# zxhuang1698/ZeroShape

Hardware: AMD Instinct MI355X
Metric: sdf_query_points_per_sec_vox128 (higher is better)
Workload: dtype f16x3

## Files before the change

### zeroshape_amd/csrc/sdf_prologue.hip

```cpp
#include "zs_common.h"
#include "sdf_layout.h"
#include "../../include/zeroshape_hip.h"

#include <math.h>

namespace {

using namespace zs::lay;

constexpr int ROWS = 4;
constexpr int LIN_THREADS = 256;
constexpr int KMAX = 1024;

__device__ __forceinline__ float wave_sum(float v) {
#pragma unroll
    for (int o = 32; o > 0; o >>= 1) v += __shfl_xor(v, o, 64);
    return v;
}

__device__ __forceinline__ float erf_ref(float x) { return erff(x); }

template <bool LN_IN, bool GELU, bool RESID, bool POS>
__global__ __launch_bounds__(LIN_THREADS) void lat_linear_kernel(
    const float *__restrict__ X, int ldx, size_t x_stride, int K, const float *__restrict__ Wt,
    const float *__restrict__ bias, int N, const float *__restrict__ ln_g,
    const float *__restrict__ ln_b, const float *__restrict__ resid, int ldr, size_t r_stride,
    const float *__restrict__ pos, float *__restrict__ Y, int ldy, size_t y_stride, int rows) {
    __shared__ float xs[ROWS][KMAX];
    const int img = blockIdx.z;
    const int r0 = blockIdx.x * ROWS;
    const int n = blockIdx.y * LIN_THREADS + threadIdx.x;
    X += (size_t)img * x_stride;
    Y += (size_t)img * y_stride;

    for (int i = threadIdx.x; i < ROWS * K; i += LIN_THREADS) {
        const int r = i / K, k = i - r * K;
        const int rr = min(r0 + r, rows - 1);
        xs[r][k] = X[(size_t)rr * ldx + k];
    }
    __syncthreads();
    if (LN_IN) {
        const int w = threadIdx.x >> 6, lane = threadIdx.x & 63;
        float v[4], s = 0.f;
#pragma unroll
        for (int j = 0; j < 4; j++) {
            v[j] = xs[w][lane + 64 * j];
            s += v[j];
        }
        const float mean = wave_sum(s) * (1.0f / 256.0f);
        float q = 0.f;
#pragma unroll
        for (int j = 0; j < 4; j++) {
            const float d = v[j] - mean;
            q = fmaf(d, d, q);
        }
        const float rstd = 1.0f / sqrtf(wave_sum(q) * (1.0f / 256.0f) + 1e-6f);
#pragma unroll
        for (int j = 0; j < 4; j++) {
            const int k = lane + 64 * j;
            xs[w][k] = fmaf((v[j] - mean) * rstd, ln_g[k], ln_b[k]);
        }
        __syncthreads();
    }
    float acc[ROWS];
#pragma unroll
    for (int r = 0; r < ROWS; r++) acc[r] = 0.f;
    for (int k0 = 0; k0 < K; k0 += 16) {
        float w[16];
#pragma unroll
        for (int j = 0; j < 16; j++) w[j] = Wt[(size_t)(k0 + j) * N + n];
#pragma unroll
        for (int j = 0; j < 16; j++)
#pragma unroll
            for (int r = 0; r < ROWS; r++) acc[r] = fmaf(xs[r][k0 + j], w[j], acc[r]);
    }
    const float b = bias[n];
#pragma unroll
    for (int r = 0; r < ROWS; r++) {
        const int row = r0 + r;
        if (row >= rows) break;
        float v = acc[r] + b;
        if (POS) v += pos[(size_t)row * N + n];
        if (GELU) v = 0.5f * v * (1.0f + erf_ref(v * 0.70710678118654752440f));
        if (RESID) v += resid[(size_t)img * r_stride + (size_t)row * ldr + n];
        Y[(size_t)row * ldy + n] = v;
    }
}

__global__ __launch_bounds__(256) void lat_self_attn_kernel(const float *__restrict__ qkv,
                                                            size_t stride, float *__restrict__ out,
                                                            size_t out_stride) {
    __shared__ float ks[L][HD];
    __shared__ float vs[L][HD];
    const int hd = blockIdx.x, img = blockIdx.y;
    qkv += (size_t)img * stride;
    out += (size_t)img * out_stride;
    for (int i = threadIdx.x; i < L * HD; i += 256) {
        const int r = i / HD, d = i - r * HD;
        ks[r][d] = qkv[(size_t)r * (3 * C) + C + hd * HD + d];
        vs[r][d] = qkv[(size_t)r * (3 * C) + 2 * C + hd * HD + d];
    }
    __syncthreads();
    const int i = threadIdx.x;
    if (i >= L) return;
    float q[HD], o[HD];
#pragma unroll
    for (int d = 0; d < HD; d++) {
        q[d] = qkv[(size_t)i * (3 * C) + hd * HD + d];
        o[d] = 0.f;
    }
    const float scale = 0.17677669529663688110f;
    float m = -INFINITY, z = 0.f;
    for (int j = 0; j < L; j++) {
        float s = 0.f;
#pragma unroll
        for (int d = 0; d < HD; d++) s = fmaf(q[d], ks[j][d], s);
        s *= scale;
        const float mn = fmaxf(m, s);
        const float a = expf(m - mn), p = expf(s - mn);
        z = fmaf(z, a, p);
#pragma unroll
        for (int d = 0; d < HD; d++) o[d] = fmaf(p, vs[j][d], o[d] * a);
        m = mn;
    }
    const float inv = 1.0f / z;
#pragma unroll
    for (int d = 0; d < HD; d++) out[(size_t)i * C + hd * HD + d] = o[d] * inv;
}

__global__ __launch_bounds__(256) void pack_kv_kernel(const float *__restrict__ scratch,
                                                      size_t scratch_stride,
                                                      float *__restrict__ programs,
                                                      size_t program_stride) {
    const int img = blockIdx.y;
    const int e = blockIdx.x * 256 + threadIdx.x;
    const int lane = e & 63;
    const int r = (e >> 6) & 15;
    const int which = (e >> 10) & 1;
    int t = e >> 11;
    const int lt = t % LT;
    t /= LT;
    const int hd = t & 7;
    const int blk = t >> 3;
    if (blk >= BLOCKS) return;
    const float *sc = scratch + (size_t)img * scratch_stride;
    const int rw = (r & 3) + 8 * (r >> 2) + 4 * (lane >> 5);
    const int lrow = 32 * lt + (which == 0 ? (lane & 31) : rw);
    const int dim = which == 0 ? rw : (lane & 31);
    float val = 0.f;
    if (lrow < L) {
        if (blk == 0)
            val = sc[S_QKV0 + (size_t)lrow * (3 * C) + (1 + which) * C + hd * HD + dim];
        else
            val = sc[S_KV1 + (size_t)lrow * (2 * C) + which * C + hd * HD + dim];
    }
    const int group = blk * G_BLOCK + hd * G_HEAD + G_QKV_HEAD + lt * 8 + which * 4 + (r >> 2);
    programs[(size_t)img * program_stride + (size_t)group * GROUP_FLOATS + lane * 4 + (r & 3)] = val;
}

template <bool LN_IN, bool GELU, bool RESID, bool POS>
void launch_linear(hipStream_t s, int batch, const float *X, int ldx, size_t x_stride, int K,
                   const float *Wt, const float *bias, int N, const float *g, const float *b,
                   const float *resid, int ldr, size_t r_stride, const float *pos, float *Y, int ldy,
                   size_t y_stride) {
    dim3 grid((L + ROWS - 1) / ROWS, N / LIN_THREADS, batch);
    hipLaunchKernelGGL((lat_linear_kernel<LN_IN, GELU, RESID, POS>), grid, dim3(LIN_THREADS), 0, s, X,
                       ldx, x_stride, K, Wt, bias, N, g, b, resid, ldr, r_stride, pos, Y, ldy,
                       y_stride, L);
}

}

__global__ __launch_bounds__(256) void verdict_stats_kernel(const float *__restrict__ got, const float *__restrict__ want, int m,
                                                            float band, float tol, float tol_occ, float *__restrict__ stats,
                                                            int *__restrict__ flags) {
    __shared__ float red[4][256];
    __shared__ int redi[2][256];
    const int b = blockIdx.x, t = threadIdx.x;
    const float *g = got + (size_t)b * m, *w = want + (size_t)b * m;
    float mx = 0.f, sum = 0.f, mw = 0.f, mo = 0.f;
    int flips = 0, bad = 0;
    for (int i = t; i < m; i += 256) {
        const float x = g[i], y = w[i];
        if (!isfinite(x) || !isfinite(y)) bad = 1;
        const float d = fabsf(x - y);
        mx = fmaxf(mx, d);
        sum += d;
        mw = fmaxf(mw, fabsf(y));
        mo = fmaxf(mo, fabsf(1.0f / (1.0f + expf(-x)) - 1.0f / (1.0f + expf(-y))));
        flips += ((x > 0.f) != (y > 0.f)) && fabsf(y) >= band;
    }
    red[0][t] = mx; red[1][t] = sum; red[2][t] = mw; red[3][t] = mo;
    redi[0][t] = flips; redi[1][t] = bad;
    __syncthreads();
    for (int o = 128; o > 0; o >>= 1) {
        if (t < o) {
            red[0][t] = fmaxf(red[0][t], red[0][t + o]);
            red[1][t] += red[1][t + o];
            red[2][t] = fmaxf(red[2][t], red[2][t + o]);
            red[3][t] = fmaxf(red[3][t], red[3][t + o]);
            redi[0][t] += redi[0][t + o];
            redi[1][t] |= redi[1][t + o];
        }
        __syncthreads();
    }
    if (t == 0) {
        const bool finite = redi[1][0] == 0;
        const float nan = __builtin_bit_cast(float, 0x7fc00000u);
        float *o = stats + (size_t)b * 5;
        o[0] = finite ? red[0][0] : nan;
        o[1] = finite ? red[1][0] / (float)m : nan;
        o[2] = finite ? red[2][0] : nan;
        o[3] = finite ? red[3][0] : nan;
        o[4] = (float)redi[0][0];
        if (flags) {
            flags[2 * b] = (finite && red[0][0] <= tol) ? 0 : 1;
            flags[2 * b + 1] = (finite && red[3][0] <= tol_occ && redi[0][0] == 0) ? 0 : 1;
        }
    }
}

extern "C" int zs_sdf_verdict_stats(const float *got, const float *want, int batch, int m, float flip_band, float tol,
                                    float tol_occ, float *stats, int *flags, void *stream) {
    if (batch < 0 || batch > 65535 || m <= 0) {
        zs::set_err("zs_sdf_verdict_stats: bad size (batch=%d m=%d)", batch, m);
        return 0;
    }
    if (batch == 0) return 1;
    if (!got || !want || !stats) {
        zs::set_err("zs_sdf_verdict_stats: null pointer");
        return 0;
    }
    hipLaunchKernelGGL(verdict_stats_kernel, dim3(batch), dim3(256), 0, static_cast<hipStream_t>(stream), got, want, m, flip_band,
                       tol, tol_occ, stats, flags);
    return zs::check_launch("zs_sdf_verdict_stats") ? 1 : 0;
}

extern "C" size_t zs_sdf_prologue_scratch_bytes(void) { return (size_t)SCRATCH_FLOATS * sizeof(float); }

extern "C" int zs_sdf_prologue(void *programs, size_t program_stride_bytes, const float *lat_params,
                               const float *latent_depth, int batch, void *scratch, void *stream) {
    return zs_sdf_prologue_ex(programs, program_stride_bytes, lat_params, latent_depth, batch, scratch, 0, stream);
}

extern "C" int zs_sdf_prologue_ex(void *programs, size_t program_stride_bytes, const float *lat_params,
                                  const float *latent_depth, int batch, void *scratch, int flags, void *stream) {
    if (flags & ~ZS_SDF_POS_PERLAYER) {
        zs::set_err("zs_sdf_prologue_ex: unknown flags 0x%x", flags);
        return 0;
    }
    if (batch < 0) {
        zs::set_err("zs_sdf_prologue: negative batch %d", batch);
        return 0;
    }
    if (batch == 0) return 1;
    if (!programs || !lat_params || !latent_depth || !scratch) {
        zs::set_err("zs_sdf_prologue: null pointer");
        return 0;
    }
    if (program_stride_bytes % 16 != 0 || program_stride_bytes < zs_sdf_program_bytes()) {
        zs::set_err("zs_sdf_prologue: bad program stride %zu", program_stride_bytes);
        return 0;
    }
    if (batch > 65535) {
        zs::set_err("zs_sdf_prologue: batch %d > 65535", batch);
        return 0;
    }
    hipStream_t s = static_cast<hipStream_t>(stream);
    const float *P = lat_params;
    float *sc = static_cast<float *>(scratch);
    const size_t ss = SCRATCH_FLOATS;
    launch_linear<false, false, false, true>(s, batch, latent_depth, C, (size_t)L * C, C, P + LQ_WLP,
                                             P + LQ_BLP, C, nullptr, nullptr, nullptr, 0, 0,
                                             P + LQ_POS, sc + S_LAT, C, ss);
    launch_linear<true, false, false, false>(s, batch, sc + S_LAT, C, ss, C, P + LQ_WQKV0,
                                             P + LQ_BQKV0, 3 * C, P + LQ_LN1G0, P + LQ_LN1B0, nullptr,
                                             0, 0, nullptr, sc + S_QKV0, 3 * C, ss);
    hipLaunchKernelGGL(lat_self_attn_kernel, dim3(HEADS, batch), dim3(256), 0, s, sc + S_QKV0, ss,
                       sc + S_ATT, ss);
    launch_linear<false, false, true, false>(s, batch, sc + S_ATT, C, ss, C, P + LQ_WPROJ0,
                                             P + LQ_BPROJ0, C, nullptr, nullptr, sc + S_LAT, C, ss,
                                             nullptr, sc + S_X1, C, ss);
    launch_linear<true, true, false, false>(s, batch, sc + S_X1, C, ss, C, P + LQ_W1, P + LQ_B1, HID,
                                            P + LQ_LN2G0, P + LQ_LN2B0, nullptr, 0, 0, nullptr,
                                            sc + S_HID, HID, ss);
    if (flags & ZS_SDF_POS_PERLAYER)
        launch_linear<false, false, true, true>(s, batch, sc + S_HID, HID, ss, HID, P + LQ_W2, P + LQ_B2,
                                                C, nullptr, nullptr, sc + S_X1, C, ss, P + LQ_POS,
                                                sc + S_X2, C, ss);
    else
        launch_linear<false, false, true, false>(s, batch, sc + S_HID, HID, ss, HID, P + LQ_W2, P + LQ_B2,
                                                 C, nullptr, nullptr, sc + S_X1, C, ss, nullptr,
                                                 sc + S_X2, C, ss);
    launch_linear<true, false, false, false>(s, batch, sc + S_X2, C, ss, C, P + LQ_WKV1, P + LQ_BKV1,
                                             2 * C, P + LQ_LN1G1, P + LQ_LN1B1, nullptr, 0, 0, nullptr,
                                             sc + S_KV1, 2 * C, ss);
    const int elems = BLOCKS * HEADS * LT * 2 * 16 * 64;
    hipLaunchKernelGGL(pack_kv_kernel, dim3((elems + 255) / 256, batch), dim3(256), 0, s, sc, ss,
                       static_cast<float *>(programs), program_stride_bytes / sizeof(float));
    return zs::check_launch("zs_sdf_prologue") ? 1 : 0;
}
```

Baseline: 84.92 million.

## Fuse latent prologue linears into three kernels with direct KV packing

Replaces the chain of separate linear launches plus a pack kernel with three kernels: a fused projection+LN+QKV kernel, a row-tiled self-attention kernel that precomputes scores and softmax factors in LDS, and a fused proj+MLP+LN+KV kernel that writes packed KV directly into the program buffer. Weight loads are double-buffered in registers. The aim is to cut launch count, intermediate scratch round-trips and the serial per-thread attention loop. The cost is heavier per-block register use, and the prologue runs once per batch, so its share of the query throughput metric may be small.

```diff
diff --git a/zeroshape_amd/csrc/sdf_prologue.hip b/zeroshape_amd/csrc/sdf_prologue.hip
--- a/zeroshape_amd/csrc/sdf_prologue.hip
+++ b/zeroshape_amd/csrc/sdf_prologue.hip
@@ -8,9 +8,23 @@
 
 using namespace zs::lay;
 
-constexpr int ROWS = 4;
+#ifndef ZS_PROLOGUE_ROWS
+#define ZS_PROLOGUE_ROWS 4
+#endif
+constexpr int ROWS = ZS_PROLOGUE_ROWS;
 constexpr int LIN_THREADS = 256;
-constexpr int KMAX = 1024;
+constexpr int ROW_BLOCKS = (L + ROWS - 1) / ROWS;
+constexpr int LROWS_REC = LT * 32;
+
+#ifndef ZS_PROLOGUE_LOADS
+#define ZS_PROLOGUE_LOADS 32
+#endif
+
+constexpr int chunk_rows(int nc) {
+    int d = 1;
+    while (2 * d * nc <= ZS_PROLOGUE_LOADS) d *= 2;
+    return d;
+}
 
 __device__ __forceinline__ float wave_sum(float v) {
 #pragma unroll
@@ -20,27 +34,10 @@
 
 __device__ __forceinline__ float erf_ref(float x) { return erff(x); }
 
-template <bool LN_IN, bool GELU, bool RESID, bool POS>
-__global__ __launch_bounds__(LIN_THREADS) void lat_linear_kernel(
-    const float *__restrict__ X, int ldx, size_t x_stride, int K, const float *__restrict__ Wt,
-    const float *__restrict__ bias, int N, const float *__restrict__ ln_g,
-    const float *__restrict__ ln_b, const float *__restrict__ resid, int ldr, size_t r_stride,
-    const float *__restrict__ pos, float *__restrict__ Y, int ldy, size_t y_stride, int rows) {
-    __shared__ float xs[ROWS][KMAX];
-    const int img = blockIdx.z;
-    const int r0 = blockIdx.x * ROWS;
-    const int n = blockIdx.y * LIN_THREADS + threadIdx.x;
-    X += (size_t)img * x_stride;
-    Y += (size_t)img * y_stride;
-
-    for (int i = threadIdx.x; i < ROWS * K; i += LIN_THREADS) {
-        const int r = i / K, k = i - r * K;
-        const int rr = min(r0 + r, rows - 1);
-        xs[r][k] = X[(size_t)rr * ldx + k];
-    }
-    __syncthreads();
-    if (LN_IN) {
-        const int w = threadIdx.x >> 6, lane = threadIdx.x & 63;
+__device__ __forceinline__ void layer_norm_rows(float (*xs)[C], const float *__restrict__ ln_g,
+                                                const float *__restrict__ ln_b) {
+    const int lane = threadIdx.x & 63;
+    for (int w = threadIdx.x >> 6; w < ROWS; w += LIN_THREADS / 64) {
         float v[4], s = 0.f;
 #pragma unroll
         for (int j = 0; j < 4; j++) {
@@ -60,113 +57,247 @@
             const int k = lane + 64 * j;
             xs[w][k] = fmaf((v[j] - mean) * rstd, ln_g[k], ln_b[k]);
         }
-        __syncthreads();
-    }
-    float acc[ROWS];
-#pragma unroll
-    for (int r = 0; r < ROWS; r++) acc[r] = 0.f;
-    for (int k0 = 0; k0 < K; k0 += 16) {
-        float w[16];
-#pragma unroll
-        for (int j = 0; j < 16; j++) w[j] = Wt[(size_t)(k0 + j) * N + n];
-#pragma unroll
-        for (int j = 0; j < 16; j++)
-#pragma unroll
-            for (int r = 0; r < ROWS; r++) acc[r] = fmaf(xs[r][k0 + j], w[j], acc[r]);
-    }
-    const float b = bias[n];
-#pragma unroll
-    for (int r = 0; r < ROWS; r++) {
-        const int row = r0 + r;
-        if (row >= rows) break;
-        float v = acc[r] + b;
-        if (POS) v += pos[(size_t)row * N + n];
-        if (GELU) v = 0.5f * v * (1.0f + erf_ref(v * 0.70710678118654752440f));
-        if (RESID) v += resid[(size_t)img * r_stride + (size_t)row * ldr + n];
-        Y[(size_t)row * ldy + n] = v;
-    }
-}
-
-__global__ __launch_bounds__(256) void lat_self_attn_kernel(const float *__restrict__ qkv,
-                                                            size_t stride, float *__restrict__ out,
-                                                            size_t out_stride) {
-    __shared__ float ks[L][HD];
+    }
+}
+
+template <int N, int D>
+__device__ __forceinline__ void load_weights(float (&w)[N / LIN_THREADS][D], const float *__restrict__ Wt, int k0) {
+#pragma unroll
+    for (int j = 0; j < D; j++)
+#pragma unroll
+        for (int c = 0; c < N / LIN_THREADS; c++) w[c][j] = Wt[(size_t)(k0 + j) * N + c * LIN_THREADS + threadIdx.x];
+}
+
+template <int K, int N, int D>
+__device__ __forceinline__ void fma_weights(float (&acc)[N / LIN_THREADS][ROWS], const float (&w)[N / LIN_THREADS][D],
+                                            const float (*xs)[K], int k0) {
+#pragma unroll
+    for (int j = 0; j < D; j++)
+#pragma unroll
+        for (int c = 0; c < N / LIN_THREADS; c++)
+#pragma unroll
+            for (int r = 0; r < ROWS; r++) acc[c][r] = fmaf(xs[r][k0 + j], w[c][j], acc[c][r]);
+}
+
+template <int K, int N>
+__device__ __forceinline__ void rows_gemm(float (&acc)[N / LIN_THREADS][ROWS], const float (*xs)[K],
+                                          const float *__restrict__ Wt) {
+    constexpr int NC = N / LIN_THREADS, D = chunk_rows(NC);
+    static_assert(N % LIN_THREADS == 0 && K % (2 * D) == 0, "rows_gemm: shape");
+#pragma unroll
+    for (int c = 0; c < NC; c++)
+#pragma unroll
+        for (int r = 0; r < ROWS; r++) acc[c][r] = 0.f;
+    float wa[NC][D], wb[NC][D];
+    load_weights<N, D>(wa, Wt, 0);
+    for (int k0 = 0; k0 < K; k0 += 2 * D) {
+        load_weights<N, D>(wb, Wt, k0 + D);
+        fma_weights<K, N, D>(acc, wa, xs, k0);
+        if (k0 + 2 * D < K) load_weights<N, D>(wa, Wt, k0 + 2 * D);
+        fma_weights<K, N, D>(acc, wb, xs, k0 + D);
+    }
+}
+
+__device__ __forceinline__ void store_kv(float *__restrict__ prog, int blk, int which, int lrow, int col, float val) {
+    const int hd = col >> 5, dim = col & 31, lt = lrow >> 5, lr = lrow & 31;
+    const int rw = which == 0 ? dim : lr;
+    const int lane = (which == 0 ? lr : dim) + 32 * ((rw >> 2) & 1);
+    const int group = blk * G_BLOCK + hd * G_HEAD + G_QKV_HEAD + lt * 8 + which * 4 + (rw >> 3);
+    prog[(size_t)group * GROUP_FLOATS + lane * 4 + (rw & 3)] = val;
+}
+
+__device__ __forceinline__ void zero_kv_tail(float *__restrict__ prog, int blk) {
+    constexpr int R0 = ROW_BLOCKS * ROWS;
+    for (int e = threadIdx.x; e < (LROWS_REC - R0) * 2 * C; e += LIN_THREADS)
+        store_kv(prog, blk, (e >> 8) & 1, R0 + (e >> 9), e & 255, 0.f);
+}
+
+__global__ __launch_bounds__(LIN_THREADS) void lat_qkv0_kernel(const float *__restrict__ latent_depth,
+                                                               const float *__restrict__ P, float *__restrict__ scratch,
+                                                               float *__restrict__ programs, size_t program_stride) {
+    __shared__ float xs[ROWS][C];
+    __shared__ float ys[ROWS][C];
+    const int img = blockIdx.y, r0 = blockIdx.x * ROWS, n = threadIdx.x;
+    const float *X = latent_depth + (size_t)img * L * C;
+    float *sc = scratch + (size_t)img * SCRATCH_FLOATS;
+    float *prog = programs + (size_t)img * program_stride;
+
+    for (int i = threadIdx.x; i < ROWS * C; i += LIN_THREADS) {
+        const int r = i / C, k = i - r * C;
+        xs[r][k] = X[(size_t)min(r0 + r, L - 1) * C + k];
+    }
+    __syncthreads();
+    {
+        float acc[1][ROWS];
+        rows_gemm<C, C>(acc, xs, P + LQ_WLP);
+        const float b = P[LQ_BLP + n];
+#pragma unroll
+        for (int r = 0; r < ROWS; r++) {
+            const int row = min(r0 + r, L - 1);
+            float v = acc[0][r] + b;
+            v += P[LQ_POS + (size_t)row * C + n];
+            ys[r][n] = v;
+            if (r0 + r < L) sc[S_LAT + (size_t)row * C + n] = v;
+        }
+    }
+    __syncthreads();
+    layer_norm_rows(ys, P + LQ_LN1G0, P + LQ_LN1B0);
+    __syncthreads();
+    float acc[3][ROWS];
+    rows_gemm<C, 3 * C>(acc, ys, P + LQ_WQKV0);
+#pragma unroll
+    for (int c = 0; c < 3; c++) {
+        const float b = P[LQ_BQKV0 + c * C + n];
+#pragma unroll
+        for (int r = 0; r < ROWS; r++) {
+            const int row = r0 + r;
+            float v = acc[c][r] + b;
+            if (row < L) sc[S_QKV0 + (size_t)row * (3 * C) + c * C + n] = v;
+            if (c > 0) store_kv(prog, 0, c - 1, row, n, row < L ? v : 0.f);
+        }
+    }
+    if (blockIdx.x == ROW_BLOCKS - 1) zero_kv_tail(prog, 0);
+}
+
+constexpr int ATT_ROWS = 8;
+
+__global__ __launch_bounds__(256) void lat_self_attn_kernel(const float *__restrict__ qkv, float *__restrict__ out) {
+    __shared__ __align__(16) float ks_pa[L * (HD + 1)];
     __shared__ float vs[L][HD];
-    const int hd = blockIdx.x, img = blockIdx.y;
-    qkv += (size_t)img * stride;
-    out += (size_t)img * out_stride;
+    __shared__ float qs[ATT_ROWS][HD];
+    __shared__ float ss[ATT_ROWS][L];
+    static_assert(ATT_ROWS * L * 2 <= L * (HD + 1) && ATT_ROWS * HD == 256, "lat_self_attn_kernel: LDS reuse");
+    float(*ks)[HD + 1] = reinterpret_cast<float(*)[HD + 1]>(ks_pa);
+    float2(*pa)[L] = reinterpret_cast<float2(*)[L]>(ks_pa);
+    const int hd = blockIdx.x, i0 = blockIdx.y * ATT_ROWS, img = blockIdx.z;
+    qkv += (size_t)img * SCRATCH_FLOATS;
+    out += (size_t)img * SCRATCH_FLOATS;
     for (int i = threadIdx.x; i < L * HD; i += 256) {
         const int r = i / HD, d = i - r * HD;
         ks[r][d] = qkv[(size_t)r * (3 * C) + C + hd * HD + d];
         vs[r][d] = qkv[(size_t)r * (3 * C) + 2 * C + hd * HD + d];
     }
-    __syncthreads();
-    const int i = threadIdx.x;
-    if (i >= L) return;
-    float q[HD], o[HD];
-#pragma unroll
-    for (int d = 0; d < HD; d++) {
-        q[d] = qkv[(size_t)i * (3 * C) + hd * HD + d];
-        o[d] = 0.f;
-    }
+    {
+        const int r = threadIdx.x / HD, d = threadIdx.x - r * HD;
+        qs[r][d] = qkv[(size_t)min(i0 + r, L - 1) * (3 * C) + hd * HD + d];
+    }
+    __syncthreads();
     const float scale = 0.17677669529663688110f;
-    float m = -INFINITY, z = 0.f;
+    for (int e = threadIdx.x; e < ATT_ROWS * L; e += 256) {
+        const int i = e / L, j = e - i * L;
+        float s = 0.f;
+#pragma unroll
+        for (int d = 0; d < HD; d++) s = fmaf(qs[i][d], ks[j][d], s);
+        ss[i][j] = s;
+    }
+    __syncthreads();
+    const int w = threadIdx.x >> 6, lane = threadIdx.x & 63;
+    for (int i = w; i < ATT_ROWS; i += 4) {
+        float carry = -INFINITY;
+        for (int j0 = 0; j0 < L; j0 += 64) {
+            const int j = j0 + lane;
+            const float t = j < L ? ss[i][j] : -INFINITY;
+            const float s = t * scale;
+            float m = s;
+#pragma unroll
+            for (int o = 1; o < 64; o <<= 1) {
+                const float up = __shfl_up(m, o, 64);
+                if (lane >= o) m = fmaxf(m, up);
+            }
+            m = fmaxf(carry, m);
+            float mp = __shfl_up(m, 1, 64);
+            if (lane == 0) mp = carry;
+            const float a = expf(mp - m), p = expf(fmaf(t, scale, -m));
+            if (j < L) pa[i][j] = make_float2(p, a);
+            carry = __shfl(m, 63, 64);
+        }
+    }
+    __syncthreads();
+    const int i = threadIdx.x >> 5, d = threadIdx.x & 31;
+    float o = 0.f, z = 0.f;
     for (int j = 0; j < L; j++) {
-        float s = 0.f;
-#pragma unroll
-        for (int d = 0; d < HD; d++) s = fmaf(q[d], ks[j][d], s);
-        s *= scale;
-        const float mn = fmaxf(m, s);
-        const float a = expf(m - mn), p = expf(s - mn);
+        const float p = pa[i][j].x, a = pa[i][j].y;
         z = fmaf(z, a, p);
-#pragma unroll
-        for (int d = 0; d < HD; d++) o[d] = fmaf(p, vs[j][d], o[d] * a);
-        m = mn;
+        o = fmaf(p, vs[j][d], o * a);
     }
     const float inv = 1.0f / z;
-#pragma unroll
-    for (int d = 0; d < HD; d++) out[(size_t)i * C + hd * HD + d] = o[d] * inv;
-}
-
-__global__ __launch_bounds__(256) void pack_kv_kernel(const float *__restrict__ scratch,
-                                                      size_t scratch_stride,
-                                                      float *__restrict__ programs,
-                                                      size_t program_stride) {
-    const int img = blockIdx.y;
-    const int e = blockIdx.x * 256 + threadIdx.x;
-    const int lane = e & 63;
-    const int r = (e >> 6) & 15;
-    const int which = (e >> 10) & 1;
-    int t = e >> 11;
-    const int lt = t % LT;
-    t /= LT;
-    const int hd = t & 7;
-    const int blk = t >> 3;
-    if (blk >= BLOCKS) return;
-    const float *sc = scratch + (size_t)img * scratch_stride;
-    const int rw = (r & 3) + 8 * (r >> 2) + 4 * (lane >> 5);
-    const int lrow = 32 * lt + (which == 0 ? (lane & 31) : rw);
-    const int dim = which == 0 ? rw : (lane & 31);
-    float val = 0.f;
-    if (lrow < L) {
-        if (blk == 0)
-            val = sc[S_QKV0 + (size_t)lrow * (3 * C) + (1 + which) * C + hd * HD + dim];
-        else
-            val = sc[S_KV1 + (size_t)lrow * (2 * C) + which * C + hd * HD + dim];
-    }
-    const int group = blk * G_BLOCK + hd * G_HEAD + G_QKV_HEAD + lt * 8 + which * 4 + (r >> 2);
-    programs[(size_t)img * program_stride + (size_t)group * GROUP_FLOATS + lane * 4 + (r & 3)] = val;
-}
-
-template <bool LN_IN, bool GELU, bool RESID, bool POS>
-void launch_linear(hipStream_t s, int batch, const float *X, int ldx, size_t x_stride, int K,
-                   const float *Wt, const float *bias, int N, const float *g, const float *b,
-                   const float *resid, int ldr, size_t r_stride, const float *pos, float *Y, int ldy,
-                   size_t y_stride) {
-    dim3 grid((L + ROWS - 1) / ROWS, N / LIN_THREADS, batch);
-    hipLaunchKernelGGL((lat_linear_kernel<LN_IN, GELU, RESID, POS>), grid, dim3(LIN_THREADS), 0, s, X,
-                       ldx, x_stride, K, Wt, bias, N, g, b, resid, ldr, r_stride, pos, Y, ldy,
-                       y_stride, L);
+    if (i0 + i < L) out[(size_t)(i0 + i) * C + hd * HD + d] = o * inv;
+}
+
+template <bool POS>
+__global__ __launch_bounds__(LIN_THREADS) void lat_mlp_kv1_kernel(const float *__restrict__ P,
+                                                                  const float *__restrict__ scratch,
+                                                                  float *__restrict__ programs, size_t program_stride) {
+    __shared__ float xs[ROWS][C];
+    __shared__ float x1[ROWS][C];
+    __shared__ float hid[ROWS][HID];
+    const int img = blockIdx.y, r0 = blockIdx.x * ROWS, n = threadIdx.x;
+    const float *sc = scratch + (size_t)img * SCRATCH_FLOATS;
+    float *prog = programs + (size_t)img * program_stride;
+
+    for (int i = threadIdx.x; i < ROWS * C; i += LIN_THREADS) {
+        const int r = i / C, k = i - r * C;
+        xs[r][k] = sc[S_ATT + (size_t)min(r0 + r, L - 1) * C + k];
+    }
+    __syncthreads();
+    {
+        float acc[1][ROWS];
+        rows_gemm<C, C>(acc, xs, P + LQ_WPROJ0);
+        const float b = P[LQ_BPROJ0 + n];
+        __syncthreads();
+#pragma unroll
+        for (int r = 0; r < ROWS; r++) {
+            float v = acc[0][r] + b;
+            v += sc[S_LAT + (size_t)min(r0 + r, L - 1) * C + n];
+            x1[r][n] = v;
+            xs[r][n] = v;
+        }
+    }
+    __syncthreads();
+    layer_norm_rows(xs, P + LQ_LN2G0, P + LQ_LN2B0);
+    __syncthreads();
+    {
+        float acc[4][ROWS];
+        rows_gemm<C, HID>(acc, xs, P + LQ_W1);
+#pragma unroll
+        for (int c = 0; c < 4; c++) {
+            const float b = P[LQ_B1 + c * LIN_THREADS + n];
+#pragma unroll
+            for (int r = 0; r < ROWS; r++) {
+                float v = acc[c][r] + b;
+                v = 0.5f * v * (1.0f + erf_ref(v * 0.70710678118654752440f));
+                hid[r][c * LIN_THREADS + n] = v;
+            }
+        }
+    }
+    __syncthreads();
+    {
+        float acc[1][ROWS];
+        rows_gemm<HID, C>(acc, hid, P + LQ_W2);
+        const float b = P[LQ_B2 + n];
+#pragma unroll
+        for (int r = 0; r < ROWS; r++) {
+            float v = acc[0][r] + b;
+            if (POS) v += P[LQ_POS + (size_t)min(r0 + r, L - 1) * C + n];
+            v += x1[r][n];
+            x1[r][n] = v;
+        }
+    }
+    __syncthreads();
+    layer_norm_rows(x1, P + LQ_LN1G1, P + LQ_LN1B1);
+    __syncthreads();
+    float acc[2][ROWS];
+    rows_gemm<C, 2 * C>(acc, x1, P + LQ_WKV1);
+#pragma unroll
+    for (int c = 0; c < 2; c++) {
+        const float b = P[LQ_BKV1 + c * C + n];
+#pragma unroll
+        for (int r = 0; r < ROWS; r++) {
+            const int row = r0 + r;
+            store_kv(prog, 1, c, row, n, row < L ? acc[c][r] + b : 0.f);
+        }
+    }
+    if (blockIdx.x == ROW_BLOCKS - 1) zero_kv_tail(prog, 1);
 }
 
 }
@@ -269,34 +400,14 @@
     hipStream_t s = static_cast<hipStream_t>(stream);
     const float *P = lat_params;
     float *sc = static_cast<float *>(scratch);
-    const size_t ss = SCRATCH_FLOATS;
-    launch_linear<false, false, false, true>(s, batch, latent_depth, C, (size_t)L * C, C, P + LQ_WLP,
-                                             P + LQ_BLP, C, nullptr, nullptr, nullptr, 0, 0,
-                                             P + LQ_POS, sc + S_LAT, C, ss);
-    launch_linear<true, false, false, false>(s, batch, sc + S_LAT, C, ss, C, P + LQ_WQKV0,
-                                             P + LQ_BQKV0, 3 * C, P + LQ_LN1G0, P + LQ_LN1B0, nullptr,
-                                             0, 0, nullptr, sc + S_QKV0, 3 * C, ss);
-    hipLaunchKernelGGL(lat_self_attn_kernel, dim3(HEADS, batch), dim3(256), 0, s, sc + S_QKV0, ss,
-                       sc + S_ATT, ss);
-    launch_linear<false, false, true, false>(s, batch, sc + S_ATT, C, ss, C, P + LQ_WPROJ0,
-                                             P + LQ_BPROJ0, C, nullptr, nullptr, sc + S_LAT, C, ss,
-                                             nullptr, sc + S_X1, C, ss);
-    launch_linear<true, true, false, false>(s, batch, sc + S_X1, C, ss, C, P + LQ_W1, P + LQ_B1, HID,
-                                            P + LQ_LN2G0, P + LQ_LN2B0, nullptr, 0, 0, nullptr,
-                                            sc + S_HID, HID, ss);
+    float *prog = static_cast<float *>(programs);
+    const size_t ps = program_stride_bytes / sizeof(float);
+    hipLaunchKernelGGL(lat_qkv0_kernel, dim3(ROW_BLOCKS, batch), dim3(LIN_THREADS), 0, s, latent_depth, P, sc, prog, ps);
+    hipLaunchKernelGGL(lat_self_attn_kernel, dim3(HEADS, (L + ATT_ROWS - 1) / ATT_ROWS, batch), dim3(256), 0, s,
+                       sc + S_QKV0, sc + S_ATT);
     if (flags & ZS_SDF_POS_PERLAYER)
-        launch_linear<false, false, true, true>(s, batch, sc + S_HID, HID, ss, HID, P + LQ_W2, P + LQ_B2,
-                                                C, nullptr, nullptr, sc + S_X1, C, ss, P + LQ_POS,
-                                                sc + S_X2, C, ss);
+        hipLaunchKernelGGL(lat_mlp_kv1_kernel<true>, dim3(ROW_BLOCKS, batch), dim3(LIN_THREADS), 0, s, P, sc, prog, ps);
     else
-        launch_linear<false, false, true, false>(s, batch, sc + S_HID, HID, ss, HID, P + LQ_W2, P + LQ_B2,
-                                                 C, nullptr, nullptr, sc + S_X1, C, ss, nullptr,
-                                                 sc + S_X2, C, ss);
-    launch_linear<true, false, false, false>(s, batch, sc + S_X2, C, ss, C, P + LQ_WKV1, P + LQ_BKV1,
-                                             2 * C, P + LQ_LN1G1, P + LQ_LN1B1, nullptr, 0, 0, nullptr,
-                                             sc + S_KV1, 2 * C, ss);
-    const int elems = BLOCKS * HEADS * LT * 2 * 16 * 64;
-    hipLaunchKernelGGL(pack_kv_kernel, dim3((elems + 255) / 256, batch), dim3(256), 0, s, sc, ss,
-                       static_cast<float *>(programs), program_stride_bytes / sizeof(float));
+        hipLaunchKernelGGL(lat_mlp_kv1_kernel<false>, dim3(ROW_BLOCKS, batch), dim3(LIN_THREADS), 0, s, P, sc, prog, ps);
     return zs::check_launch("zs_sdf_prologue") ? 1 : 0;
 }
```

Measured after the change: 85.19 million, median of 6. No clear change (+0.3%).
